# nep-pack/NonlinearEigenproblems.jl

Hardware: AMD Instinct MI355X
Metric: eigenpairs/sec (gun SPMF iar m=100) + compute_Mlincomb GB/s (higher is better)
Workload: dtype f64 (complex128)

## Files before the change

### nonlineareigenproblems.jl_amd/csrc/driver.hip

```cpp
#include "common.h"
#include <vector>
#include <stdlib.h>
#include <time.h>

struct nep_iar {
    nep_spmf* spmf; nep_lu* lu;
    int64_t n, ldv; int32_t m, mt;
    cplx* dV; const cplx* dCtab; int64_t ldc; const int64_t* d_active;
    cplx* dz; cplx* dW;
    std::vector<double> cabs; std::vector<nep_cdouble> cf;
    cplx* dH; nep_cdouble* hH;
    double* d_cabs; cplx* d_ccf;
    cplx* hH_dev;
    int32_t method;
    std::vector<hipEvent_t> ev;
    hipEvent_t e_upload = nullptr; bool upload_waited = false;
    hipStream_t last = nullptr;
    bool no_events = false;
    std::vector<hipGraphExec_t> graphs;
    cplx* dWT = nullptr; int32_t wt_for = 0;
};

extern "C" {

int32_t nep_iar_create(nep_spmf* spmf, nep_lu* lu, int64_t n, int32_t m, nep_cdouble* dV, int64_t ldv,
                       const nep_cdouble* dCtab, int64_t ldc, const int64_t* d_active, nep_cdouble* dwork3n,
                       const double* h_cabs, const nep_cdouble* h_cf, int32_t mt, nep_cdouble* dH, nep_cdouble* h_pinnedH,
                       int32_t orth_method, nep_iar** out) {
    ARGCHK(out != nullptr);
    *out = nullptr;
// ... 94 lines not shown
        rc = nep_iar_shift_scale(n, k, (const nep_cdouble*)col, (nep_cdouble*)vv, stream);
        if (rc) return rc;
    }
    cplx* mirror = s->hH_dev ? s->hH_dev + (int64_t)(k - 1) * (s->m + 4) : nullptr;
    if (s->dWT && k < s->m) {
        rc = nep_orth_dev_iar_next((const nep_cdouble*)s->dV, s->ldv, n, k, s->d_active, (nep_cdouble*)vv, (nep_cdouble*)hrow, s->method,
                                   (nep_cdouble*)mirror, k + 4, (const nep_cdouble*)s->dCtab, s->ldc, s->mt,
                                   (nep_cdouble*)s->dWT, (nep_cdouble*)(vv + s->ldv + n), stream);
        if (!rc) s->wt_for = k + 1;
    } else
        rc = nep_orth_dev_mirror((const nep_cdouble*)s->dV, s->ldv, n * (int64_t)(k + 1), k, s->d_active, (nep_cdouble*)vv,
                                 (nep_cdouble*)hrow, s->method, (nep_cdouble*)mirror, k + 4, stream);
    if (rc) return rc;
    if (!mirror)
        HIPCHK(hipMemcpyAsync(s->hH + (int64_t)(k - 1) * (s->m + 4), hrow, (size_t)(k + 4) * sizeof(cplx), hipMemcpyDeviceToHost, st));
    if (s->no_events) return NEP_OK;
    if (!s->ev[k]) HIPCHK(hipEventCreateWithFlags(&s->ev[k], hipEventDisableTiming | hipEventBlockingSync));
    HIPCHK(hipEventRecord(s->ev[k], st));
    return NEP_OK;
}

int32_t nep_iar_steps(nep_iar* s, int32_t k0, int32_t count, int32_t refine_steps, nep_stream stream) {
    ARGCHK(s && count >= 1);
    for (int32_t k = k0; k < k0 + count; ++k) {
        int rc = nep_iar_step(s, k, refine_steps, stream);
        if (rc) return rc;
    }
    return NEP_OK;
}

int32_t nep_iar_steps_graph(nep_iar* s, int32_t k0, int32_t count, int32_t refine_steps, nep_stream stream, int32_t* captured) {
    ARGCHK(s && count >= 1);
    if (captured) *captured = 0;
// ... 8 lines not shown
        hipGraph_t g = nullptr;
        hipError_t e = hipStreamEndCapture(st, &g);
        hipGraphExec_t ge = nullptr;
        if (!rc && e == hipSuccess && g && hipGraphInstantiate(&ge, g, nullptr, nullptr, 0) == hipSuccess && ge) {
            if (hipGraphLaunch(ge, st) == hipSuccess) { s->graphs.push_back(ge); ok = true; }
            else (void)hipGraphExecDestroy(ge);
        }
        if (g) (void)hipGraphDestroy(g);
        if (!ok) (void)hipGetLastError();
    } else (void)hipGetLastError();
    if (!ok) {
        s->wt_for = wt_for0; s->upload_waited = waited0; s->last = last0;
        return nep_iar_steps(s, k0, count, refine_steps, stream);
    }
    for (int32_t k = k0; k < k0 + count; ++k) {
        if (!s->ev[k]) HIPCHK(hipEventCreateWithFlags(&s->ev[k], hipEventDisableTiming | hipEventBlockingSync));
        HIPCHK(hipEventRecord(s->ev[k], st));
    }
    if (captured) *captured = 1;
    return NEP_OK;
}

int32_t nep_iar_wait(nep_iar* s, int32_t k) {
    ARGCHK(s && k >= 1 && k <= s->m && s->ev[k]);
    for (;;) {
        const hipError_t e = hipEventQuery(s->ev[k]);
        if (e == hipSuccess) return NEP_OK;
        if (e != hipErrorNotReady) HIPCHK(e);
        struct timespec ts = {0, 20000};
        nanosleep(&ts, nullptr);
// ... 11 lines not shown
```

### nonlineareigenproblems.jl_amd/csrc/hesseig.hip

```cpp
#include "common.h"
#include <math.h>

namespace {

constexpr double HQ_ULP = 2.220446049250313e-16;
constexpr double HQ_SAFMIN = 2.2250738585072014e-308;
constexpr int HQ_KMAX = 128;

__host__ __device__ __forceinline__ int hq_off(int c) { return (c * (c + 3)) >> 1; }
__host__ __device__ __forceinline__ int hq_entries(int k) { return hq_off(k - 1) + k; }
__device__ __forceinline__ double cabs1(cplx z) { return fabs(z.x) + fabs(z.y); }
__device__ __forceinline__ cplx readlane_c(cplx v, int lane) { return cmake(readlane_d(v.x, lane), readlane_d(v.y, lane)); }
__device__ __forceinline__ cplx cconj(cplx a) { return cmake(a.x, -a.y); }
__device__ __forceinline__ cplx czero() { return cmake(0.0, 0.0); }

__device__ __forceinline__ double rsqrt_nr(double x) {
    const double y = __builtin_amdgcn_rsq(x);
    const double e = fma(-(x * y), y, 1.0);
    const double q = fma(0.375, e, 0.5);
    return fma(y * e, q, y);
}
__device__ __forceinline__ double rcp_nr(double x) {
    double y = __builtin_amdgcn_rcp(x);
    double e = fma(-x, y, 1.0);
// ... 51 lines not shown
        const double sup = cabs1(A[hq_off(kk) + kk - 1]);
        const double ab = fmax(sub, sup), ba = fmin(sub, sup);
        const double a2 = cabs1(d2), dd = cabs1(csub(d1, d2));
        const double aa = fmax(a2, dd), bb = fmin(a2, dd);
        const double is = rcp_nr(aa + ab);
        if (ba * (ab * is) <= fmax(smlnum, HQ_ULP * (bb * (aa * is)))) return true;
    }
    return false;
}

struct HqCtl {
    int seq;
    int l, i;
    int prog;
    int rq_done;
    int pad[3];
    double tx, ty;
};
typedef __attribute__((address_space(3))) volatile int lds_vint;
typedef __attribute__((address_space(3))) volatile double lds_vdbl;
__device__ __forceinline__ int ctl_load(const int* p) { return *(lds_vint*)p; }
__device__ __forceinline__ void ctl_store(int* p, int v) { *(lds_vint*)p = v; }
__device__ __forceinline__ double ctl_loadd(const double* p) { return *(lds_vdbl*)p; }
__device__ __forceinline__ void ctl_stored(double* p, double v) { *(lds_vdbl*)p = v; }
#define HQ_CBAR() asm volatile("" ::: "memory")

#define HQ_APPLY(c_, s_, up_, lo_, nu_, nl_)                                                                          \
    cplx nu_ = cscale(c_, up_); cfma(nu_, s_, lo_);                                                                   \
    cplx nl_ = cscale(c_, lo_); cfma(nl_, cmake(-(s_).x, (s_).y), up_)

template <bool TWO>
__device__ __forceinline__ void qr_half(cplx* A, cplx* rot, int* prog, const int ld, const int l, const int i,
                                        const int lane) {
    const int c0 = l + lane;
    if (!TWO) {
        const bool in0 = c0 <= i;
        cplx* col = A + hq_off(in0 ? c0 : i);
        cplx up = col[l], lo = col[l + 1];
        cplx lon = col[l + 2];
        double c; cplx s;
        lartg_n(readlane_c(up, 0), readlane_c(lo, 0), c, s);
        cplx pnu, ps; double pc;
        { HQ_APPLY(c, s, up, lo, nu, nl); pnu = nu; pc = c; ps = s; up = nl; lo = lon; }
        for (int j = l + 2; j <= i; ++j) {
            lon = col[j + 1];
            if (in0 && c0 + 2 >= j) col[j - 2] = pnu;
            rot[2 * (j - 1)] = cmake(pc, 0.0); rot[2 * (j - 1) + 1] = ps;
            HQ_CBAR(); ctl_store(prog, j); HQ_CBAR();
// ... 38 lines not shown
        for (int j = jm + 1; j <= i; ++j) {
            lo1n = col1[j + 1];
            if (in1 && c1 + 2 >= j) col1[j - 2] = pnu1;
            rot[2 * (j - 1)] = cmake(pc, 0.0); rot[2 * (j - 1) + 1] = ps;
            HQ_CBAR(); ctl_store(prog, j); HQ_CBAR();
            const int gl = j - 1 - l - 64;
            lartg_n(readlane_c(up1, gl), readlane_c(lo1, gl), c, s);
            HQ_APPLY(c, s, up1, lo1, nu1, nl1);
            pnu1 = nu1; pc = c; ps = s;
            up1 = nl1; lo1 = lo1n;
        }
        if (in1 && c1 + 2 >= i + 1) col1[i - 1] = pnu1;
        rot[2 * i] = cmake(pc, 0.0); rot[2 * i + 1] = ps;
        if (c1 == i) col1[i] = up1;
    }
    HQ_CBAR(); ctl_store(prog, i + 2); HQ_CBAR();
}

#define HQ_RQ(c_, s_, y_, z_, o_, n_)                                                                                 \
    cplx o_ = cscale(c_, y_); cfma_conj(o_, s_, z_);                                              \
    cplx n_ = cscale(c_, z_); cfma(n_, cmake(-(s_).x, -(s_).y), y_)
#define HQ_WAIT(need_)                                                                                                \
    while (pc_ < (need_)) { pc_ = ctl_load(prog); if (pc_ < (need_)) __builtin_amdgcn_s_sleep(1); }                    \
    HQ_CBAR()

template <bool TWO>
__device__ __forceinline__ void rq_half(cplx* A, const cplx* rot, const int* prog, const int ld, const int l, const int i,
                                        const cplx t, const int lane) {
    const int r0 = l + lane;
    int pc_ = 0;
    HQ_WAIT(l + 3);
    if (!TWO) {
        const bool in0 = r0 <= i;
        const int r0c = in0 ? r0 : i;
        cplx y = (lane == 0) ? A[hq_off(l) + l] : czero();
        for (int j = l + 1; j <= i; ++j) {
            HQ_WAIT(j + 2);
            cplx z = A[hq_off(j) + r0c];
            const double c = rot[2 * j].x; const cplx s = rot[2 * j + 1];
            if (r0 > j) z = czero();
            HQ_RQ(c, s, y, z, o, ny);
            if (r0 == j - 1) o = cadd(o, t);
            if (in0 && r0 <= j) A[hq_off((j - 1)) + r0] = o;
            y = ny;
        }
        if (in0) { if (r0 == i) y = cadd(y, t); A[hq_off(i) + r0] = y; }
    } else {
        const int r1 = r0 + 64;
        const bool in1 = r1 <= i;
        const int r1c = in1 ? r1 : i;
        cplx y0 = (lane == 0) ? A[hq_off(l) + l] : czero(), y1 = czero();
        const int jm = l + 63;
        for (int j = l + 1; j <= jm; ++j) {
            HQ_WAIT(j + 2);
            cplx z0 = A[hq_off(j) + r0];
            const double c = rot[2 * j].x; const cplx s = rot[2 * j + 1];
            if (r0 > j) z0 = czero();
            HQ_RQ(c, s, y0, z0, o, ny);
            if (r0 == j - 1) o = cadd(o, t);
            if (r0 <= j) A[hq_off((j - 1)) + r0] = o;
            y0 = ny;
        }
        for (int j = jm + 1; j <= i; ++j) {
            HQ_WAIT(j + 2);
            const cplx z0 = A[hq_off(j) + r0];
            cplx z1 = A[hq_off(j) + r1c];
            const double c = rot[2 * j].x; const cplx s = rot[2 * j + 1];
            if (r1 > j) z1 = czero();
            HQ_RQ(c, s, y0, z0, o0, n0);
            HQ_RQ(c, s, y1, z1, o1, n1);
            if (r0 == j - 1) o0 = cadd(o0, t);
            if (r1 == j - 1) o1 = cadd(o1, t);
            A[hq_off((j - 1)) + r0] = o0;
            if (in1 && r1 <= j) A[hq_off((j - 1)) + r1] = o1;
            y0 = n0; y1 = n1;
        }
        A[hq_off(i) + r0] = y0;
        if (in1) { if (r1 == i) y1 = cadd(y1, t); A[hq_off(i) + r1] = y1; }
    }
}

struct HessWork { cplx* Ht; cplx* wk; cplx* misc; cplx* U; };
__device__ __host__ inline HessWork hq_carve(void* d_work, int k) {
    HessWork W; cplx* p = (cplx*)d_work;
    W.Ht = p; p += (size_t)k * k; W.wk = p; p += k; W.misc = p; p += 2; W.U = p;
    return W;
}

__global__ __launch_bounds__(128) void k_hess_qr(int k0, int kstep, const cplx* __restrict__ H, int64_t ldh, cplx* __restrict__ w_base,
                                                 int64_t w_stride, char* __restrict__ work_base, int64_t work_stride,
                                                 cplx* __restrict__ mirror_base, int64_t mirror_stride) {
    const int k = k0 + (int)blockIdx.x * kstep;
    cplx* __restrict__ w_out = w_base + (size_t)blockIdx.x * w_stride;
    const HessWork Wk = hq_carve(work_base + (size_t)blockIdx.x * work_stride, k);
    cplx* __restrict__ Ht = Wk.Ht; cplx* __restrict__ wk_out = Wk.wk; cplx* __restrict__ misc = Wk.misc;
    cplx* __restrict__ mirror = mirror_base ? mirror_base + (size_t)blockIdx.x * mirror_stride : nullptr;
    extern __shared__ cplx sm[];
    cplx* A = sm;
    cplx* rot = sm + hq_entries(k);
    HqCtl* ctl = (HqCtl*)(rot + 2 * (k + 1));
    const int lane = threadIdx.x & 63;
    const int wave = __builtin_amdgcn_readfirstlane(threadIdx.x >> 6);
    const int ld = k;
    if (threadIdx.x == 0) { ctl->seq = 0; ctl->prog = 0; ctl->rq_done = 0; ctl->l = 0; ctl->i = 0; ctl->tx = 0.0; ctl->ty = 0.0; }
    __syncthreads();
    if (wave == 1) {
        int myseq = 0;
        for (;;) {
            int sq;
            while ((sq = ctl_load(&ctl->seq)) == myseq) __builtin_amdgcn_s_sleep(1);
            HQ_CBAR();
            if (sq < 0) break;
            myseq = sq;
            const int lw = __builtin_amdgcn_readfirstlane(ctl_load(&ctl->l)), iw = __builtin_amdgcn_readfirstlane(ctl_load(&ctl->i));
            const cplx t = cmake(ctl_loadd(&ctl->tx), ctl_loadd(&ctl->ty));
            if (iw - lw + 1 > 64) rq_half<true>(A, rot, &ctl->prog, ld, lw, iw, t, lane);
            else rq_half<false>(A, rot, &ctl->prog, ld, lw, iw, t, lane);
            HQ_CBAR();
            ctl_store(&ctl->rq_done, myseq);
            HQ_CBAR();
        }
        __syncthreads();
        __syncthreads();
        return;
    }
    double amax = 0.0;
    for (int c = 0; c < k; ++c) {
        const int rl = c + 1 < k - 1 ? c + 1 : k - 1;
        for (int r = lane; r <= rl; r += 64) {
            const cplx v = H[(size_t)c * ldh + r];
            A[hq_off(c) + r] = v;
            amax = fmax(amax, fmax(fabs(v.x), fabs(v.y)));
// ... 63 lines not shown
                    cplx y = cscale(s, csqrt_fast(cadd(cmul(xs, xs), cmul(us, us))));
                    if (sx > 0.0 && (x.x * y.x + x.y * y.y) < 0.0) y = cmake(-y.x, -y.y);
                    const cplx den = cadd(x, y);
                    if (den.x != 0.0 || den.y != 0.0) t = csub(t, cmul(u, cdiv_fast(u, den)));
                }
            }
            const int lw = __builtin_amdgcn_readfirstlane(l), iw = __builtin_amdgcn_readfirstlane(i);
            TP(tq3);
            {
                const int d0 = lw + lane, d1 = d0 + 64;
                if (d0 <= iw) A[hq_off(d0) + d0] = csub(A[hq_off(d0) + d0], t);
                if (d1 <= iw) A[hq_off(d1) + d1] = csub(A[hq_off(d1) + d1], t);
            }
            ++seq;
            HQ_CBAR();
            ctl_store(&ctl->prog, 0); ctl_store(&ctl->l, lw); ctl_store(&ctl->i, iw);
            ctl_stored(&ctl->tx, t.x); ctl_stored(&ctl->ty, t.y);
            HQ_CBAR();
            ctl_store(&ctl->seq, seq);
            HQ_CBAR();
            TP(tq4);
            if (iw - lw + 1 > 64) qr_half<true>(A, rot, &ctl->prog, ld, lw, iw, lane);
            else qr_half<false>(A, rot, &ctl->prog, ld, lw, iw, lane);
#ifdef HQ_PROF
            { const long long tq5 = clock64(); tp_wait += tq1 - tq0; tp_scan += tq2 - tq1; tp_shift += tq3 - tq2; tp_pub += tq4 - tq3; tp_qr += tq5 - tq4; tp_steps += iw - lw; }
#endif
        }
        if (!conv) { info = i + 1; break; }
        i = __builtin_amdgcn_readfirstlane(l - 1);
    }
    while (ctl_load(&ctl->rq_done) != seq) __builtin_amdgcn_s_sleep(1);
    HQ_CBAR();
    ctl_store(&ctl->seq, -1);
    HQ_CBAR();
    __syncthreads();
    cplx* wk = rot;
    for (int e = lane; e < k; e += 64) {
        cplx we = czero();
        if (info == 0) { we = A[hq_off(e) + e]; we = cmake(ldexp(we.x, sexp), ldexp(we.y, sexp)); }
        wk[e] = we; w_out[e] = we;
        if (mirror) mirror[e] = we;
    }
    if (info == 0) {
        for (int e = 1; e < k; ++e) {
            for (int guard = 0; guard < 4 * k; ++guard) {
                const cplx we = wk[e];
                bool close = false;
                for (int q = lane; q < e; q += 64) close = close || (cabs1(csub(wk[q], we)) < eps3);
// ... 177 lines not shown
    return NEP_OK;
}

int32_t nep_hess_eigvals_batch_dev(int32_t nb, int32_t k0, int32_t kstep, const nep_cdouble* dH, int64_t ldh, nep_cdouble* d_w,
                                   int64_t w_stride, void* d_work, int64_t work_stride, nep_cdouble* h_mirror,
                                   int64_t mirror_stride, nep_stream stream) {
    ARGCHK(nb >= 1 && k0 >= 1 && kstep >= 0 && dH && d_w && d_work);
    const int kmax = k0 + (nb - 1) * kstep;
    ARGCHK(ldh >= kmax);
    if (kmax > HQ_KMAX) { nep_set_error("nep_hess_eigvals_dev: k = %d exceeds the LDS-resident limit %d", kmax, HQ_KMAX); return NEP_ERR_UNSUPPORTED; }
    if (nb > 1) {
        int64_t need = 0; int rcw = nep_hess_eig_worksize(kmax, &need); if (rcw) return rcw;
        ARGCHK(w_stride >= kmax + 2 && work_stride >= need && (work_stride % 16) == 0 && (!h_mirror || mirror_stride >= kmax + 2));
    }
    const size_t lds = (size_t)16 * hq_entries(kmax) + (size_t)32 * (kmax + 1) + 48;
    if (lds > 65536) { int rc = nep_raise_lds((const void*)k_hess_qr, 163840); if (rc) return rc; }
    cplx* mir = mapped(h_mirror);
    if (h_mirror && !mir) { nep_set_error("nep_hess_eigvals_dev: h_mirror is not mapped pinned host memory"); return NEP_ERR_ARG; }
    hipLaunchKernelGGL(k_hess_qr, dim3((unsigned)nb), dim3(128), lds, as_stream(stream), (int)k0, (int)kstep, (const cplx*)dH, ldh,
                       (cplx*)d_w, w_stride, (char*)d_work, work_stride, mir, mirror_stride);
    LAUNCHCHK();
    return NEP_OK;
}

int32_t nep_hess_eigvecs_batch_dev(int32_t nb, int32_t k0, int32_t kstep, nep_cdouble* d_w, int64_t w_stride, nep_cdouble* dZ,
                                   int64_t ldz, int64_t z_stride, void* d_work, int64_t work_stride, nep_cdouble* h_mirror,
                                   int64_t mirror_stride, nep_stream stream) {
    ARGCHK(nb >= 1 && k0 >= 1 && kstep >= 0 && d_w && dZ && d_work);
    const int kmax = k0 + (nb - 1) * kstep;
    ARGCHK(kmax <= HQ_KMAX && ldz >= kmax && (nb == 1 || z_stride >= (int64_t)kmax * ldz));
    cplx* mir = mapped(h_mirror);
    if (h_mirror && !mir) { nep_set_error("nep_hess_eigvecs_dev: h_mirror is not mapped pinned host memory"); return NEP_ERR_ARG; }
    hipLaunchKernelGGL(k_hess_invit, dim3((unsigned)kmax, (unsigned)nb), dim3(64), 0, as_stream(stream), (int)k0, (int)kstep,
                       (cplx*)d_w, w_stride, (char*)d_work, work_stride, (cplx*)dZ, ldz, z_stride, mir, mirror_stride);
    LAUNCHCHK();
// ... 15 lines not shown
```

### nonlineareigenproblems.jl_amd/csrc/iar_run.hip

```cpp
#include "common.h"
#include <algorithm>
#include <deque>
#include <map>
#include <mutex>
#include <vector>
#include <math.h>
#include <time.h>

extern "C" {
int32_t nep_iar_create(nep_spmf* spmf, nep_lu* lu, int64_t n, int32_t m, nep_cdouble* dV, int64_t ldv, const nep_cdouble* dCtab,
                       int64_t ldc, const int64_t* d_active, nep_cdouble* dwork3n, const double* h_cabs, const nep_cdouble* h_cf,
                       int32_t mt, nep_cdouble* dH, nep_cdouble* h_pinnedH, int32_t orth_method, nep_iar** out);
int32_t nep_iar_steps_graph(nep_iar* s, int32_t k0, int32_t count, int32_t refine_steps, nep_stream stream, int32_t* captured);
}

namespace {

constexpr double EPS = 2.220446049250313e-16;

__global__ void k_iar_active(int64_t* act, int64_t n, int m1) {
    const int j = blockIdx.x * blockDim.x + threadIdx.x;
    if (j < m1) act[j] = (int64_t)(j + 1) * n;
}
__global__ void k_iar_start(cplx* __restrict__ V, const cplx* __restrict__ v, double inv, int64_t n) {
    const int64_t i = (int64_t)blockIdx.x * blockDim.x + threadIdx.x;
    if (i < n) V[i] = cmake(v[i].x * inv, v[i].y * inv);
}

constexpr int64_t ZSLACK = 8192;
__global__ __launch_bounds__(256) void k_iar_zero_slack(cplx* __restrict__ V, int64_t ldv, int64_t n, int m1) {
    const int j = blockIdx.y;
    const int64_t a = (int64_t)(j + 1) * n;
    const int64_t r = a + (int64_t)blockIdx.x * 256 + threadIdx.x;
    if (j < m1 && r < ldv && r < a + ZSLACK) V[(int64_t)j * ldv + r] = cmake(0.0, 0.0);
}

struct RunStreams { hipStream_t check = nullptr, eig = nullptr; hipStream_t probed_for = (hipStream_t)-1; bool shared = false; int retries = 0; };
std::mutex g_rs_mu;
std::map<int, RunStreams> g_rs;

constexpr int RUN_STREAM_CANDIDATES = 8;
int pick_stream(hipStream_t keep, const std::vector<hipStream_t>& others, hipStream_t* out, bool* shared) {
    const int prio = 0, ncand = RUN_STREAM_CANDIDATES;
    std::vector<hipStream_t> cand;
    if (keep) cand.push_back(keep);
    hipStream_t pick = nullptr;
    for (int c = 0; c < ncand && !pick; ++c) {
        hipStream_t s = nullptr;
        if ((size_t)c < cand.size()) s = cand[c];
        else { HIPCHK(hipStreamCreateWithPriority(&s, hipStreamNonBlocking, prio)); cand.push_back(s); }
        bool clash = false;
        for (size_t i = 0; i < others.size() && !clash; ++i) {
            int32_t a = 0;
            int rc = nep_stream_pair_serializes((nep_stream)others[i], (nep_stream)s, &a); if (rc) return rc;
            clash = a != 0;
        }
        if (!clash) pick = s;
    }
    if (getenv("NEP_IAR_RUN_TRACE")) fprintf(stderr, "nep_iar_run: stream pick (prio %d): %zu candidates tried, %s\n", prio, cand.size(), pick ? "free queue found" : "none free");
    if (!pick) { pick = cand[0]; *shared = true; }
    for (hipStream_t s : cand) if (s != pick) (void)hipStreamDestroy(s);
    *out = pick;
    return NEP_OK;
}

int run_streams(hipStream_t main, RunStreams* out) {
    int dev = 0; HIPCHK(hipGetDevice(&dev));
    std::lock_guard<std::mutex> lk(g_rs_mu);
    RunStreams& r = g_rs[dev];
    if (!r.check || !r.eig || r.probed_for != main || (r.shared && r.retries < 3)) {
        if (r.shared) ++r.retries;
        r.shared = false;
        int rc = pick_stream(r.check, {main}, &r.check, &r.shared); if (rc) return rc;
        rc = pick_stream(r.eig, {main, r.check}, &r.eig, &r.shared); if (rc) return rc;
        r.probed_for = main;
    }
    *out = r;
    return NEP_OK;
}

struct Arena {
    int dev = -1; int64_t n = 0; int32_t m = 0, mt = 0;
    cplx* Hdev = nullptr; cplx* wdev = nullptr; cplx* Ctab = nullptr; cplx* work3n = nullptr; int64_t* active = nullptr;
    cplx* v0 = nullptr; double* d_norms = nullptr; void* eigwork = nullptr; int64_t wsz = 0; int bmax = 0;
    cplx* Hpin = nullptr; cplx* wpin = nullptr; double* npin = nullptr; cplx* stage = nullptr;
    void release() {
        for (void* p : {(void*)Hdev, (void*)wdev, (void*)Ctab, (void*)work3n, (void*)active, (void*)v0, (void*)d_norms, eigwork})
            if (p) nep_pool_free(p);
        for (void* p : {(void*)Hpin, (void*)wpin, (void*)npin, (void*)stage}) if (p) (void)hipHostFree(p);
        *this = Arena();
    }
};
std::mutex g_arena_mu;
std::vector<Arena> g_arenas;

int arena_acquire(int64_t n, int32_t m, int32_t mt, int bmax, Arena* out) {
    int dev = 0; HIPCHK(hipGetDevice(&dev));
    {
        std::lock_guard<std::mutex> lk(g_arena_mu);
        for (size_t i = 0; i < g_arenas.size(); ++i)
            if (g_arenas[i].dev == dev && g_arenas[i].n == n && g_arenas[i].m == m && g_arenas[i].mt == mt && g_arenas[i].bmax == bmax) {
                *out = g_arenas[i]; g_arenas.erase(g_arenas.begin() + i); return NEP_OK;
            }
    }
    Arena a; a.dev = dev; a.n = n; a.m = m; a.mt = mt; a.bmax = bmax;
    int64_t wsz = 0; int rc = nep_hess_eig_worksize(m, &wsz); if (rc) return rc;
    a.wsz = (wsz + 15) / 16 * 16;
    void* p = nullptr;
#define AL(dst, type, bytes) do { rc = nep_pool_alloc(&p, (size_t)(bytes)); if (rc) { a.release(); return rc; } dst = (type)p; } while (0)
    AL(a.Hdev, cplx*, (size_t)m * (m + 4) * 16);
    AL(a.wdev, cplx*, (size_t)m * (m + 2) * 16);
    AL(a.Ctab, cplx*, (size_t)m * mt * 16);
    AL(a.work3n, cplx*, (size_t)3 * n * 16);
    AL(a.active, int64_t*, (size_t)(m + 1) * 8);
    AL(a.v0, cplx*, (size_t)n * 16);
    AL(a.d_norms, double*, (size_t)m * 2 * m * 8);
    AL(a.eigwork, void*, (size_t)bmax * a.wsz);
#undef AL
    const size_t stage_bytes = std::max<size_t>((size_t)n * 16, (size_t)m * mt * 16);
    if (hipHostMalloc((void**)&a.Hpin, (size_t)m * (m + 4) * 16, hipHostMallocMapped) != hipSuccess ||
        hipHostMalloc((void**)&a.wpin, (size_t)m * (m + 2) * 16, hipHostMallocMapped) != hipSuccess ||
        hipHostMalloc((void**)&a.npin, (size_t)m * 2 * m * 8, hipHostMallocDefault) != hipSuccess ||
        hipHostMalloc((void**)&a.stage, stage_bytes, hipHostMallocDefault) != hipSuccess) {
        (void)hipGetLastError(); a.release();
        nep_set_error("nep_iar_run: pinned host allocation failed");
        return NEP_ERR_HIP;
    }
    *out = a;
    return NEP_OK;
}
void arena_return(Arena& a) {
    std::lock_guard<std::mutex> lk(g_arena_mu);
// ... 29 lines not shown
            const double om = w[step];
            if (om <= 2.0 * EPS) { ret = step; break; }
            if (om > 0.5 * w_prev) { ret = om > w_prev ? step - 1 : step; break; }
            if (step == umf) { ret = step; break; }
            w_prev = om;
        }
        if (ret < 0) ret = plan;
        last_omega = w[plan];
        recorded = std::max(ret, 1);
        const bool ok = isfinite(w[plan]) && (ret == plan || w[plan] <= std::max(4.0 * EPS, w[ret]));
        if (ok) { if (!hint_off) hint = recorded; } else { hint = -1; hint_off = true; }
        return ok;
    }
};

struct Batch { std::vector<int> kcs; cplx* Zb = nullptr; int kmax = 0; hipEvent_t evW = nullptr, evZ = nullptr; };
struct Check { int kc = 0; std::vector<double> lam; cplx* QT = nullptr; std::vector<double> F; hipEvent_t ev = nullptr; cplx* Zb_owner = nullptr; };

inline cplx hc(const nep_cdouble& z) { cplx r; r.x = z.re; r.y = z.im; return r; }
inline bool ev_done(hipEvent_t e) {
    if (hipEventQuery(e) == hipSuccess) return true;
    (void)hipGetLastError();
    return false;
}

struct Run {
    nep_spmf* spmf; nep_lu* lu; int64_t n; nep_iar_opts o; nep_fv_eval fv; void* ctx; const double* h_fro;
    hipStream_t st; RunStreams rs; Arena a; bool have_arena = false;
    int32_t m, mt; int64_t ldv;
    cplx* V = nullptr; bool own_V = true; nep_iar* step = nullptr;
    Refine ref;
// ... 61 lines not shown
                    const nep_cdouble* h_Ctab, int32_t mt, const double* h_cabs, const nep_cdouble* h_cf, const double* h_fro,
                    nep_fv_eval fv, void* ctx, nep_cdouble* h_lam, nep_cdouble* dQ, nep_cdouble* h_Q, double* h_err,
                    nep_cdouble* dV_basis, nep_iar_result* res, nep_stream stream) {
    ARGCHK(spmf && lu && opts && h_v0 && h_Ctab && fv && h_lam && res);
    ARGCHK(n > 0 && mt >= 1 && opts->maxit >= 1 && opts->check_error_every >= 1);
    ARGCHK(opts->orth_method == 0 || opts->orth_method == 1);
    ARGCHK(opts->errmeasure == 0 || (opts->errmeasure == 1 && h_fro));
    ARGCHK(opts->umfpack_refinements <= 0 || (h_cabs && h_cf));
    memset(res, 0, sizeof(*res));
    res->refine_plan = -1;
    struct timespec t_e_; clock_gettime(CLOCK_MONOTONIC, &t_e_);
    const double t_entry = t_e_.tv_sec * 1e3 + t_e_.tv_nsec * 1e-6;
    const int32_t m = opts->maxit;
    if (m > 128) { nep_set_error("nep_iar_run: maxit = %d exceeds the device eigen-decomposition's limit 128", m); return NEP_ERR_UNSUPPORTED; }
    const int BMAX = std::max(1, nep_env_int("NEP_IAR_EIG_BATCH", 16));
    const int LASTB = std::max(1, nep_env_int("NEP_IAR_EIG_LAST", 8));
    const double T100 = nep_env_double("NEP_IAR_EIG_MS100", 3.3);
    const double TSTEP = 0.35;
    const int cee = opts->check_error_every;
    const double neigs = opts->neigs;
    const bool unthrottled = isinf(neigs) && neigs > 0;

    Run R; R.spmf = spmf; R.lu = lu; R.n = n; R.o = *opts; R.fv = fv; R.ctx = ctx; R.h_fro = h_fro; R.st = as_stream(stream);
    R.m = m; R.mt = mt; R.ldv = n * (int64_t)(m + 1); R.h_err = h_err;
    int rc = run_streams(R.st, &R.rs); if (rc) return rc;
    rc = arena_acquire(n, m, mt, BMAX, &R.a); if (rc) return rc;
    R.have_arena = true;
    Arena& a = R.a;
    hipStream_t st = R.st, cst = R.rs.check, est = R.rs.eig;
    R.ref.umf = opts->umfpack_refinements > 0 ? opts->umfpack_refinements : 0;
    R.ref.hint = (opts->refine_hint >= 0 && nep_env_int("NEP_REFINE_HINT", 1) != 0) ? opts->refine_hint : -1;
    R.filled.assign(m + 1, 0); R.plans.assign(m + 1, 0);
    if (const char* fa = getenv("NEP_IAR_RUN_FAIL_AT")) { if (sscanf(fa, "%d:%d", &R.fail_kind, &R.fail_at) != 2) R.fail_kind = R.fail_at = 0; }
    if (h_err) for (int64_t i = 0; i < (int64_t)m * m; ++i) h_err[i] = NAN;

    if (dV_basis) { R.V = (cplx*)dV_basis; R.own_V = false; }
    else {
        void* p = nullptr;
        rc = nep_pool_alloc(&p, (size_t)(m + 1) * R.ldv * 16); if (rc) return rc;
        R.V = (cplx*)p;
    }
    double nrm2 = 0.0;
    for (int64_t i = 0; i < n; ++i) { a.stage[i] = hc(h_v0[i]); nrm2 += h_v0[i].re * h_v0[i].re + h_v0[i].im * h_v0[i].im; }
    ARGCHK(nrm2 > 0.0 && isfinite(nrm2));
// ... 19 lines not shown
                        (nep_cdouble*)a.Hpin, opts->orth_method, &R.step);
    if (rc) return rc;

    std::vector<char> plan_end(m + 2, 0);
    if (unthrottled) {
        std::vector<int> allk;
        for (int kk = 1; kk <= m; ++kk) if (kk % cee == 0 || kk == m) allk.push_back(kk);
        int e_ = (int)allk.size(); int size = std::min(LASTB, e_);
        while (e_ > 0) {
            plan_end[allk[e_ - 1]] = 1; e_ -= size;
            if (e_ > 0) {
                const double q = allk[e_ - 1] / 100.0;
                size = (int)std::min<double>(std::min(BMAX, e_), std::max(1.0, ceil(2.0 * T100 * q * q / (TSTEP * cee))));
            }
        }
    }
    const bool trace = getenv("NEP_IAR_RUN_TRACE") != nullptr;
    auto now = []() { struct timespec t; clock_gettime(CLOCK_MONOTONIC, &t); return t.tv_sec * 1e3 + t.tv_nsec * 1e-6; };
    double t_fv = 0;
    std::deque<int> pendA; std::deque<Batch> stA; std::deque<Check> stC;
    int slots = unthrottled ? m + 1 : std::max(BMAX, 4);
    const int CHUNK = unthrottled ? 8 : 4;
    const int P = std::min(256, std::max(1, 3072 / mt));
    int k = 1; bool done = false; int status = NEP_OK;
    const bool use_graph = nep_env_flag("NEP_IAR_GRAPH");
    int n_graph = 0;
    auto finished = [&]() { return R.conv >= neigs; };

    auto batch_ready = [&]() -> int {
        if (pendA.empty()) return 0;
        int cnt = 1;
        while (cnt < (int)pendA.size() && cnt < BMAX && pendA[cnt] - pendA[cnt - 1] == pendA[1] - pendA[0] && !(unthrottled && plan_end[pendA[cnt - 1]])) ++cnt;
        if (!unthrottled || plan_end[pendA[cnt - 1]] || cnt >= BMAX || done) return cnt;
        return 0;
    };
    auto launch_batch = [&](int count) -> int {
        Batch b;
        for (int i = 0; i < count; ++i) { b.kcs.push_back(pendA.front()); pendA.pop_front(); }
        const int k0 = b.kcs[0], nb = count; b.kmax = b.kcs.back();
        const int kstep = nb > 1 ? b.kcs[1] - k0 : 0;
        int r = nep_iar_stream_wait(R.step, b.kmax, (nep_stream)est); if (r) return r;
        cplx* wrow = a.wdev + (int64_t)(k0 - 1) * (m + 2);
        cplx* mrow = a.wpin + (int64_t)(k0 - 1) * (m + 2);
        r = nep_hess_eigvals_batch_dev(nb, k0, kstep, (const nep_cdouble*)a.Hdev, m + 4, (nep_cdouble*)wrow, (int64_t)kstep * (m + 2),
                                       a.eigwork, a.wsz, (nep_cdouble*)mrow, (int64_t)kstep * (m + 2), (nep_stream)est);
        if (r) return r;
        b.evW = R.event(); if (!b.evW) return NEP_ERR_HIP;
        HIPCHK(hipEventRecord(b.evW, est));
        void* pz = nullptr;
        r = nep_pool_alloc(&pz, (size_t)nb * b.kmax * b.kmax * 16); if (r) return r;
        b.Zb = (cplx*)pz;
        r = nep_hess_eigvecs_batch_dev(nb, k0, kstep, (nep_cdouble*)wrow, (int64_t)kstep * (m + 2), (nep_cdouble*)b.Zb, b.kmax,
                                       (int64_t)b.kmax * b.kmax, a.eigwork, a.wsz, (nep_cdouble*)mrow, (int64_t)kstep * (m + 2), (nep_stream)est);
        if (r) { nep_pool_free_on(b.Zb, est, true); return r; }
        b.evZ = R.event(); if (!b.evZ) return NEP_ERR_HIP;
        HIPCHK(hipEventRecord(b.evZ, est));
        stA.push_back(b);
        return NEP_OK;
    };
    auto launch_check = [&](const Batch& b, int bi, bool first_of_batch) -> int {
        const int kc = b.kcs[bi];
        int r = R.fill_H(kc); if (r) return r;
        const cplx* w = a.wpin + (int64_t)(kc - 1) * (m + 2);
        if (w[kc].x != 0.0 || (R.fail_kind == 3 && R.fail_at == kc)) { R.retry = 3; nep_set_error("nep_iar_run: the QR iteration of step %d gave up", kc); return NEP_ERR_RETRY; }
        Check c; c.kc = kc; c.lam.resize(2 * (size_t)kc); c.F.resize(2 * (size_t)mt * kc);
        const double sr = R.o.sigma.re, si = R.o.sigma.im, gr = R.o.gamma.re, gi = R.o.gamma.im;
        for (int s = 0; s < kc; ++s) {
            const double dr = w[s].x, di = w[s].y, den = dr * dr + di * di;
// ... 60 lines not shown
            R.s_lam[2 * s] = c.lam[2 * src]; R.s_lam[2 * s + 1] = c.lam[2 * src + 1];
        }
        if (!(kc == m || conv >= neigs)) for (int s = 0; s < nret; ++s) R.s_idx[s] = idx[s];
        if (R.s_QT) nep_pool_free_on(R.s_QT, cst, true);
        R.s_QT = c.QT; c.QT = nullptr; R.s_kq = kc;
        R.conv = conv; R.k_checked = kc;
        R.done(c.ev); c.ev = nullptr;
        return NEP_OK;
    };
    auto drop_check = [&](Check& c) {
        if (c.QT) nep_pool_free_on(c.QT, cst, true);
        if (c.Zb_owner) nep_pool_free_on(c.Zb_owner, cst, true);
        R.done(c.ev);
    };
    auto drop_batch = [&](Batch& b) {
        if (b.Zb) nep_pool_free_on(b.Zb, est, true);
        R.done(b.evW); R.done(b.evZ);
    };

    hipEvent_t te0 = nullptr, te1 = nullptr; bool te1_rec = false;
    if (trace) { (void)hipEventCreate(&te0); (void)hipEventCreate(&te1); (void)hipEventRecord(te0, st); }
    const double t_loop = now();
    double tt_steps = 0, tt_A = 0, tt_B = 0, tt_C = 0, tt_sleep = 0, t_enq_done = 0; double tq = 0;
    while (status == NEP_OK) {
        bool progressed = false;
        tq = now();
        if (!done) {
            if (k <= m && !finished()) {
                int nb = 0;
                while (nb < CHUNK && k + nb <= m) {
                    const bool due = ((k + nb) % cee == 0) || (k + nb == m);
// ... 45 lines not shown
            if (status) { drop_check(c); break; }
        }
        if (status) break;
        if (finished()) {
            done = true; pendA.clear();
            while (!stA.empty()) { drop_batch(stA.front()); stA.pop_front(); }
            while (!stC.empty()) { drop_check(stC.front()); stC.pop_front(); }
        }
        if (trace) { const double t = now(); tt_C += t - tq; tq = t; }
        if (done && pendA.empty() && stA.empty() && stC.empty()) break;
        if (!progressed) { struct timespec ts = {0, 20000}; nanosleep(&ts, nullptr); if (trace) { const double t = now(); tt_sleep += t - tq; tq = t; } }
    }
    if (trace)
        fprintf(stderr, "nep_iar_run trace (ms): set-up %.2f | loop %.2f: steps %.2f (all enqueued at %.2f) A %.2f B %.2f (callback %.2f) C %.2f sleep %.2f\n",
                t_loop - t_entry, now() - t_loop, tt_steps, t_enq_done, tt_A, tt_B, t_fv, tt_C, tt_sleep);
    if (trace && use_graph) fprintf(stderr, "nep_iar_run: %d chunks went out as hipGraphs\n", n_graph);
    if (trace && te0 && te1 && te1_rec) {
        float ms_ = 0.0f;
        if (hipEventSynchronize(te1) == hipSuccess && hipEventElapsedTime(&ms_, te0, te1) == hipSuccess)
            fprintf(stderr, "nep_iar_run: the recurrence's %d steps took %.2f ms on the device\n", m, ms_);
        (void)hipGetLastError();
    }
    if (te0) (void)hipEventDestroy(te0);
    if (te1) (void)hipEventDestroy(te1);
    while (!stA.empty()) { drop_batch(stA.front()); stA.pop_front(); }
    while (!stC.empty()) { drop_check(stC.front()); stC.pop_front(); }
    (void)hipStreamSynchronize(est);
    (void)hipStreamSynchronize(cst);
    res->retry_reason = R.retry;
    res->refine_plan = R.ref.hint_off ? -1 : (R.ref.recorded >= 0 ? R.ref.recorded : R.ref.hint);
    res->refine_hint_off = R.ref.hint_off ? 1 : 0;
    if (status || !unthrottled) (void)hipStreamSynchronize(st);
    if (status) return status;

    int nret = (int)(R.s_lam.size() / 2);
    const bool noconv = (R.conv < neigs) && !unthrottled;
    if (!noconv) nret = std::min(nret, R.conv);
    res->k = R.k_checked > 0 ? R.k_checked : k - 1;
    res->nconv = R.conv; res->nret = nret;
    for (int s = 0; s < nret; ++s) { h_lam[s].re = R.s_lam[2 * s]; h_lam[s].im = R.s_lam[2 * s + 1]; }
    if (nret > 0 && (dQ || h_Q) && R.s_QT) {
        cplx* dst = (cplx*)dQ; void* tmp = nullptr;
// ... 16 lines not shown
```

Baseline: 1417.

## Split Hessenberg QR sweep across four waves and add second eigen stream

The Hessenberg QR kernel gains a four-wave variant. A third wave runs the upper 64-column half of each QR sweep in a pipeline behind the first wave, using a second progress word that the RQ wave waits on. The final eigen-decomposition batch (the one ending at m) now runs on a separate stream with its own workspace, so it can overlap earlier batches, and the default last batch size drops. Per-step event recording is also limited to the steps where a check plan ends, which cuts event overhead. In exchange the kernel carries more inter-wave synchronisation and the arena allocates a larger eigen workspace.

```diff
diff --git a/nonlineareigenproblems.jl_amd/csrc/driver.hip b/nonlineareigenproblems.jl_amd/csrc/driver.hip
--- a/nonlineareigenproblems.jl_amd/csrc/driver.hip
+++ b/nonlineareigenproblems.jl_amd/csrc/driver.hip
@@ -14,6 +14,7 @@
     cplx* hH_dev;
     int32_t method;
     std::vector<hipEvent_t> ev;
+    std::vector<char> ev_steps;
     hipEvent_t e_upload = nullptr; bool upload_waited = false;
     hipStream_t last = nullptr;
     bool no_events = false;
@@ -138,9 +139,15 @@
     if (rc) return rc;
     if (!mirror)
         HIPCHK(hipMemcpyAsync(s->hH + (int64_t)(k - 1) * (s->m + 4), hrow, (size_t)(k + 4) * sizeof(cplx), hipMemcpyDeviceToHost, st));
-    if (s->no_events) return NEP_OK;
+    if (s->no_events || (!s->ev_steps.empty() && !s->ev_steps[k])) return NEP_OK;
     if (!s->ev[k]) HIPCHK(hipEventCreateWithFlags(&s->ev[k], hipEventDisableTiming | hipEventBlockingSync));
     HIPCHK(hipEventRecord(s->ev[k], st));
+    return NEP_OK;
+}
+
+int32_t nep_iar_event_steps(nep_iar* s, const char* steps) {
+    ARGCHK(s && steps);
+    s->ev_steps.assign(steps, steps + s->m + 1);
     return NEP_OK;
 }
 
@@ -179,6 +186,7 @@
         return nep_iar_steps(s, k0, count, refine_steps, stream);
     }
     for (int32_t k = k0; k < k0 + count; ++k) {
+        if (!s->ev_steps.empty() && !s->ev_steps[k]) continue;
         if (!s->ev[k]) HIPCHK(hipEventCreateWithFlags(&s->ev[k], hipEventDisableTiming | hipEventBlockingSync));
         HIPCHK(hipEventRecord(s->ev[k], st));
     }
diff --git a/nonlineareigenproblems.jl_amd/csrc/hesseig.hip b/nonlineareigenproblems.jl_amd/csrc/hesseig.hip
--- a/nonlineareigenproblems.jl_amd/csrc/hesseig.hip
+++ b/nonlineareigenproblems.jl_amd/csrc/hesseig.hip
@@ -89,7 +89,9 @@
     int l, i;
     int prog;
     int rq_done;
-    int pad[3];
+    int prog2;
+    int seq2;
+    int pad;
     double tx, ty;
 };
 typedef __attribute__((address_space(3))) volatile int lds_vint;
@@ -106,7 +108,7 @@
 
 template <bool TWO>
 __device__ __forceinline__ void qr_half(cplx* A, cplx* rot, int* prog, const int ld, const int l, const int i,
-                                        const int lane) {
+                                        const int fin, const int lane) {
     const int c0 = l + lane;
     if (!TWO) {
         const bool in0 = c0 <= i;
@@ -175,28 +177,65 @@
         rot[2 * i] = cmake(pc, 0.0); rot[2 * i + 1] = ps;
         if (c1 == i) col1[i] = up1;
     }
-    HQ_CBAR(); ctl_store(prog, i + 2); HQ_CBAR();
+    HQ_CBAR(); ctl_store(prog, fin); HQ_CBAR();
+}
+
+#define HQ_WAIT(word_, need_)                                                                                         \
+    while (pc_ < (need_)) { pc_ = ctl_load(word_); if (pc_ < (need_)) __builtin_amdgcn_s_sleep(1); }                   \
+    HQ_CBAR()
+
+__device__ __forceinline__ void qr_upper(cplx* A, cplx* rot, const int* prog0, int* prog2, const int l, const int i,
+                                         const int lane) {
+    const int c1 = l + 64 + lane;
+    const bool in1 = c1 <= i;
+    cplx* col1 = A + hq_off(in1 ? c1 : i);
+    cplx up1 = col1[l], lo1 = col1[l + 1], lo1n = col1[l + 2];
+    int pc_ = 0;
+    HQ_WAIT(prog0, l + 2);
+    double c = rot[2 * (l + 1)].x; cplx s = rot[2 * (l + 1) + 1];
+    cplx pnu1, ps; double pc;
+    { HQ_APPLY(c, s, up1, lo1, nu1, nl1); pnu1 = nu1; pc = c; ps = s; up1 = nl1; lo1 = lo1n; }
+    const int jm = l + 64;
+    for (int j = l + 2; j <= jm; ++j) {
+        lo1n = col1[j + 1];
+        if (in1) col1[j - 2] = pnu1;
+        HQ_WAIT(prog0, j + 1);
+        c = rot[2 * j].x; s = rot[2 * j + 1];
+        HQ_APPLY(c, s, up1, lo1, nu1, nl1);
+        pnu1 = nu1; pc = c; ps = s; up1 = nl1; lo1 = lo1n;
+    }
+    for (int j = jm + 1; j <= i; ++j) {
+        lo1n = col1[j + 1];
+        if (in1 && c1 + 2 >= j) col1[j - 2] = pnu1;
+        rot[2 * (j - 1)] = cmake(pc, 0.0); rot[2 * (j - 1) + 1] = ps;
+        HQ_CBAR(); ctl_store(prog2, j); HQ_CBAR();
+        const int gl = j - 1 - l - 64;
+        lartg_n(readlane_c(up1, gl), readlane_c(lo1, gl), c, s);
+        HQ_APPLY(c, s, up1, lo1, nu1, nl1);
+        pnu1 = nu1; pc = c; ps = s;
+        up1 = nl1; lo1 = lo1n;
+    }
+    if (in1 && c1 + 2 >= i + 1) col1[i - 1] = pnu1;
+    rot[2 * i] = cmake(pc, 0.0); rot[2 * i + 1] = ps;
+    if (c1 == i) col1[i] = up1;
+    HQ_CBAR(); ctl_store(prog2, i + 2); HQ_CBAR();
 }
 
 #define HQ_RQ(c_, s_, y_, z_, o_, n_)                                                                                 \
     cplx o_ = cscale(c_, y_); cfma_conj(o_, s_, z_);                                              \
     cplx n_ = cscale(c_, z_); cfma(n_, cmake(-(s_).x, -(s_).y), y_)
-#define HQ_WAIT(need_)                                                                                                \
-    while (pc_ < (need_)) { pc_ = ctl_load(prog); if (pc_ < (need_)) __builtin_amdgcn_s_sleep(1); }                    \
-    HQ_CBAR()
-
-template <bool TWO>
-__device__ __forceinline__ void rq_half(cplx* A, const cplx* rot, const int* prog, const int ld, const int l, const int i,
-                                        const cplx t, const int lane) {
+template <bool TWO, bool FOUR>
+__device__ __forceinline__ void rq_half(cplx* A, const cplx* rot, const int* prog, const int* prog2, const int ld, const int l,
+                                        const int i, const cplx t, const int lane) {
     const int r0 = l + lane;
     int pc_ = 0;
-    HQ_WAIT(l + 3);
+    HQ_WAIT(prog, l + 3);
     if (!TWO) {
         const bool in0 = r0 <= i;
         const int r0c = in0 ? r0 : i;
         cplx y = (lane == 0) ? A[hq_off(l) + l] : czero();
         for (int j = l + 1; j <= i; ++j) {
-            HQ_WAIT(j + 2);
+            HQ_WAIT(prog, j + 2);
             cplx z = A[hq_off(j) + r0c];
             const double c = rot[2 * j].x; const cplx s = rot[2 * j + 1];
             if (r0 > j) z = czero();
@@ -213,7 +252,7 @@
         cplx y0 = (lane == 0) ? A[hq_off(l) + l] : czero(), y1 = czero();
         const int jm = l + 63;
         for (int j = l + 1; j <= jm; ++j) {
-            HQ_WAIT(j + 2);
+            HQ_WAIT(prog, j + 2);
             cplx z0 = A[hq_off(j) + r0];
             const double c = rot[2 * j].x; const cplx s = rot[2 * j + 1];
             if (r0 > j) z0 = czero();
@@ -222,8 +261,10 @@
             if (r0 <= j) A[hq_off((j - 1)) + r0] = o;
             y0 = ny;
         }
+        const int* progb = FOUR ? prog2 : prog;
+        if (FOUR) { HQ_WAIT(prog, i + 2); pc_ = 0; }
         for (int j = jm + 1; j <= i; ++j) {
-            HQ_WAIT(j + 2);
+            HQ_WAIT(progb, j + 2);
             const cplx z0 = A[hq_off(j) + r0];
             cplx z1 = A[hq_off(j) + r1c];
             const double c = rot[2 * j].x; const cplx s = rot[2 * j + 1];
@@ -248,9 +289,11 @@
     return W;
 }
 
-__global__ __launch_bounds__(128) void k_hess_qr(int k0, int kstep, const cplx* __restrict__ H, int64_t ldh, cplx* __restrict__ w_base,
-                                                 int64_t w_stride, char* __restrict__ work_base, int64_t work_stride,
-                                                 cplx* __restrict__ mirror_base, int64_t mirror_stride) {
+template <int WAVES>
+__global__ __launch_bounds__(64 * WAVES) void k_hess_qr(int k0, int kstep, const cplx* __restrict__ H, int64_t ldh, cplx* __restrict__ w_base,
+                                                        int64_t w_stride, char* __restrict__ work_base, int64_t work_stride,
+                                                        cplx* __restrict__ mirror_base, int64_t mirror_stride) {
+    constexpr bool FOUR = WAVES == 4;
     const int k = k0 + (int)blockIdx.x * kstep;
     cplx* __restrict__ w_out = w_base + (size_t)blockIdx.x * w_stride;
     const HessWork Wk = hq_carve(work_base + (size_t)blockIdx.x * work_stride, k);
@@ -263,8 +306,28 @@
     const int lane = threadIdx.x & 63;
     const int wave = __builtin_amdgcn_readfirstlane(threadIdx.x >> 6);
     const int ld = k;
-    if (threadIdx.x == 0) { ctl->seq = 0; ctl->prog = 0; ctl->rq_done = 0; ctl->l = 0; ctl->i = 0; ctl->tx = 0.0; ctl->ty = 0.0; }
+    if (threadIdx.x == 0) {
+        ctl->seq = 0; ctl->prog = 0; ctl->rq_done = 0; ctl->l = 0; ctl->i = 0; ctl->tx = 0.0; ctl->ty = 0.0;
+        ctl->prog2 = 0; ctl->seq2 = 0;
+    }
     __syncthreads();
+    if (FOUR && wave >= 2) {
+        if (wave == 2 && k > 64) {
+            int myseq = 0;
+            for (;;) {
+                int sq;
+                while ((sq = ctl_load(&ctl->seq2)) == myseq) __builtin_amdgcn_s_sleep(2);
+                HQ_CBAR();
+                if (sq < 0) break;
+                myseq = sq;
+                const int lw = __builtin_amdgcn_readfirstlane(ctl_load(&ctl->l)), iw = __builtin_amdgcn_readfirstlane(ctl_load(&ctl->i));
+                qr_upper(A, rot, &ctl->prog, &ctl->prog2, lw, iw, lane);
+            }
+        }
+        __syncthreads();
+        __syncthreads();
+        return;
+    }
     if (wave == 1) {
         int myseq = 0;
         for (;;) {
@@ -275,8 +338,8 @@
             myseq = sq;
             const int lw = __builtin_amdgcn_readfirstlane(ctl_load(&ctl->l)), iw = __builtin_amdgcn_readfirstlane(ctl_load(&ctl->i));
             const cplx t = cmake(ctl_loadd(&ctl->tx), ctl_loadd(&ctl->ty));
-            if (iw - lw + 1 > 64) rq_half<true>(A, rot, &ctl->prog, ld, lw, iw, t, lane);
-            else rq_half<false>(A, rot, &ctl->prog, ld, lw, iw, t, lane);
+            if (iw - lw + 1 > 64) rq_half<true, FOUR>(A, rot, &ctl->prog, &ctl->prog2, ld, lw, iw, t, lane);
+            else rq_half<false, false>(A, rot, &ctl->prog, &ctl->prog2, ld, lw, iw, t, lane);
             HQ_CBAR();
             ctl_store(&ctl->rq_done, myseq);
             HQ_CBAR();
@@ -370,14 +433,18 @@
             }
             ++seq;
             HQ_CBAR();
+            const bool wide = iw - lw + 1 > 64;
             ctl_store(&ctl->prog, 0); ctl_store(&ctl->l, lw); ctl_store(&ctl->i, iw);
+            if (FOUR) ctl_store(&ctl->prog2, 0);
             ctl_stored(&ctl->tx, t.x); ctl_stored(&ctl->ty, t.y);
             HQ_CBAR();
+            if (FOUR && wide) ctl_store(&ctl->seq2, seq);
             ctl_store(&ctl->seq, seq);
             HQ_CBAR();
             TP(tq4);
-            if (iw - lw + 1 > 64) qr_half<true>(A, rot, &ctl->prog, ld, lw, iw, lane);
-            else qr_half<false>(A, rot, &ctl->prog, ld, lw, iw, lane);
+            if (!wide) qr_half<false>(A, rot, &ctl->prog, ld, lw, iw, iw + 2, lane);
+            else if (FOUR) qr_half<false>(A, rot, &ctl->prog, ld, lw, lw + 64, iw + 2, lane);
+            else qr_half<true>(A, rot, &ctl->prog, ld, lw, iw, iw + 2, lane);
 #ifdef HQ_PROF
             { const long long tq5 = clock64(); tp_wait += tq1 - tq0; tp_scan += tq2 - tq1; tp_shift += tq3 - tq2; tp_pub += tq4 - tq3; tp_qr += tq5 - tq4; tp_steps += iw - lw; }
 #endif
@@ -388,6 +455,7 @@
     while (ctl_load(&ctl->rq_done) != seq) __builtin_amdgcn_s_sleep(1);
     HQ_CBAR();
     ctl_store(&ctl->seq, -1);
+    if (FOUR) ctl_store(&ctl->seq2, -1);
     HQ_CBAR();
     __syncthreads();
     cplx* wk = rot;
@@ -595,11 +663,19 @@
         ARGCHK(w_stride >= kmax + 2 && work_stride >= need && (work_stride % 16) == 0 && (!h_mirror || mirror_stride >= kmax + 2));
     }
     const size_t lds = (size_t)16 * hq_entries(kmax) + (size_t)32 * (kmax + 1) + 48;
-    if (lds > 65536) { int rc = nep_raise_lds((const void*)k_hess_qr, 163840); if (rc) return rc; }
+    const int waves = nep_env_int("NEP_HESS_QR_WAVES", 4);
+    if (waves != 2 && waves != 4) { nep_set_error("NEP_HESS_QR_WAVES = %d: 2 or 4", waves); return NEP_ERR_ARG; }
+    const bool four = waves == 4 && kmax > 64;
+    const void* kern = four ? (const void*)k_hess_qr<4> : (const void*)k_hess_qr<2>;
+    if (lds > 65536) { int rc = nep_raise_lds(kern, 163840); if (rc) return rc; }
     cplx* mir = mapped(h_mirror);
     if (h_mirror && !mir) { nep_set_error("nep_hess_eigvals_dev: h_mirror is not mapped pinned host memory"); return NEP_ERR_ARG; }
-    hipLaunchKernelGGL(k_hess_qr, dim3((unsigned)nb), dim3(128), lds, as_stream(stream), (int)k0, (int)kstep, (const cplx*)dH, ldh,
-                       (cplx*)d_w, w_stride, (char*)d_work, work_stride, mir, mirror_stride);
+    if (four)
+        hipLaunchKernelGGL(k_hess_qr<4>, dim3((unsigned)nb), dim3(256), lds, as_stream(stream), (int)k0, (int)kstep, (const cplx*)dH, ldh,
+                           (cplx*)d_w, w_stride, (char*)d_work, work_stride, mir, mirror_stride);
+    else
+        hipLaunchKernelGGL(k_hess_qr<2>, dim3((unsigned)nb), dim3(128), lds, as_stream(stream), (int)k0, (int)kstep, (const cplx*)dH, ldh,
+                           (cplx*)d_w, w_stride, (char*)d_work, work_stride, mir, mirror_stride);
     LAUNCHCHK();
     return NEP_OK;
 }
diff --git a/nonlineareigenproblems.jl_amd/csrc/iar_run.hip b/nonlineareigenproblems.jl_amd/csrc/iar_run.hip
--- a/nonlineareigenproblems.jl_amd/csrc/iar_run.hip
+++ b/nonlineareigenproblems.jl_amd/csrc/iar_run.hip
@@ -12,6 +12,7 @@
                        int64_t ldc, const int64_t* d_active, nep_cdouble* dwork3n, const double* h_cabs, const nep_cdouble* h_cf,
                        int32_t mt, nep_cdouble* dH, nep_cdouble* h_pinnedH, int32_t orth_method, nep_iar** out);
 int32_t nep_iar_steps_graph(nep_iar* s, int32_t k0, int32_t count, int32_t refine_steps, nep_stream stream, int32_t* captured);
+int32_t nep_iar_event_steps(nep_iar* s, const char* steps);
 }
 
 namespace {
@@ -35,7 +36,10 @@
     if (j < m1 && r < ldv && r < a + ZSLACK) V[(int64_t)j * ldv + r] = cmake(0.0, 0.0);
 }
 
-struct RunStreams { hipStream_t check = nullptr, eig = nullptr; hipStream_t probed_for = (hipStream_t)-1; bool shared = false; int retries = 0; };
+struct RunStreams {
+    hipStream_t check = nullptr, eig = nullptr, eig2 = nullptr; hipStream_t probed_for = (hipStream_t)-1; bool shared = false; int retries = 0;
+    bool eig2_probed = false;
+};
 std::mutex g_rs_mu;
 std::map<int, RunStreams> g_rs;
 
@@ -64,17 +68,23 @@
     return NEP_OK;
 }
 
-int run_streams(hipStream_t main, RunStreams* out) {
+int run_streams(hipStream_t main, bool want_eig2, RunStreams* out) {
     int dev = 0; HIPCHK(hipGetDevice(&dev));
     std::lock_guard<std::mutex> lk(g_rs_mu);
     RunStreams& r = g_rs[dev];
     if (!r.check || !r.eig || r.probed_for != main || (r.shared && r.retries < 3)) {
         if (r.shared) ++r.retries;
-        r.shared = false;
+        r.shared = false; r.eig2_probed = false;
         int rc = pick_stream(r.check, {main}, &r.check, &r.shared); if (rc) return rc;
         rc = pick_stream(r.eig, {main, r.check}, &r.eig, &r.shared); if (rc) return rc;
         r.probed_for = main;
     }
+    if (want_eig2 && !r.eig2_probed) {
+        bool sh2 = false;
+        int rc = pick_stream(r.eig2, {main, r.check, r.eig}, &r.eig2, &sh2); if (rc) return rc;
+        if (sh2) { (void)hipStreamDestroy(r.eig2); r.eig2 = nullptr; }
+        r.eig2_probed = true;
+    }
     *out = r;
     return NEP_OK;
 }
@@ -82,7 +92,7 @@
 struct Arena {
     int dev = -1; int64_t n = 0; int32_t m = 0, mt = 0;
     cplx* Hdev = nullptr; cplx* wdev = nullptr; cplx* Ctab = nullptr; cplx* work3n = nullptr; int64_t* active = nullptr;
-    cplx* v0 = nullptr; double* d_norms = nullptr; void* eigwork = nullptr; int64_t wsz = 0; int bmax = 0;
+    cplx* v0 = nullptr; double* d_norms = nullptr; void* eigwork = nullptr; int64_t wsz = 0; int bmax = 0, nsets = 0;
     cplx* Hpin = nullptr; cplx* wpin = nullptr; double* npin = nullptr; cplx* stage = nullptr;
     void release() {
         for (void* p : {(void*)Hdev, (void*)wdev, (void*)Ctab, (void*)work3n, (void*)active, (void*)v0, (void*)d_norms, eigwork})
@@ -94,16 +104,16 @@
 std::mutex g_arena_mu;
 std::vector<Arena> g_arenas;
 
-int arena_acquire(int64_t n, int32_t m, int32_t mt, int bmax, Arena* out) {
+int arena_acquire(int64_t n, int32_t m, int32_t mt, int bmax, int nsets, Arena* out) {
     int dev = 0; HIPCHK(hipGetDevice(&dev));
     {
         std::lock_guard<std::mutex> lk(g_arena_mu);
         for (size_t i = 0; i < g_arenas.size(); ++i)
-            if (g_arenas[i].dev == dev && g_arenas[i].n == n && g_arenas[i].m == m && g_arenas[i].mt == mt && g_arenas[i].bmax == bmax) {
+            if (g_arenas[i].dev == dev && g_arenas[i].n == n && g_arenas[i].m == m && g_arenas[i].mt == mt && g_arenas[i].bmax == bmax && g_arenas[i].nsets == nsets) {
                 *out = g_arenas[i]; g_arenas.erase(g_arenas.begin() + i); return NEP_OK;
             }
     }
-    Arena a; a.dev = dev; a.n = n; a.m = m; a.mt = mt; a.bmax = bmax;
+    Arena a; a.dev = dev; a.n = n; a.m = m; a.mt = mt; a.bmax = bmax; a.nsets = nsets;
     int64_t wsz = 0; int rc = nep_hess_eig_worksize(m, &wsz); if (rc) return rc;
     a.wsz = (wsz + 15) / 16 * 16;
     void* p = nullptr;
@@ -115,7 +125,7 @@
     AL(a.active, int64_t*, (size_t)(m + 1) * 8);
     AL(a.v0, cplx*, (size_t)n * 16);
     AL(a.d_norms, double*, (size_t)m * 2 * m * 8);
-    AL(a.eigwork, void*, (size_t)bmax * a.wsz);
+    AL(a.eigwork, void*, (size_t)nsets * bmax * a.wsz);
 #undef AL
     const size_t stage_bytes = std::max<size_t>((size_t)n * 16, (size_t)m * mt * 16);
     if (hipHostMalloc((void**)&a.Hpin, (size_t)m * (m + 4) * 16, hipHostMallocMapped) != hipSuccess ||
@@ -175,7 +185,7 @@
     }
 };
 
-struct Batch { std::vector<int> kcs; cplx* Zb = nullptr; int kmax = 0; hipEvent_t evW = nullptr, evZ = nullptr; };
+struct Batch { std::vector<int> kcs; cplx* Zb = nullptr; int kmax = 0; hipEvent_t evW = nullptr, evZ = nullptr; hipStream_t es = nullptr; };
 struct Check { int kc = 0; std::vector<double> lam; cplx* QT = nullptr; std::vector<double> F; hipEvent_t ev = nullptr; cplx* Zb_owner = nullptr; };
 
 inline cplx hc(const nep_cdouble& z) { cplx r; r.x = z.re; r.y = z.im; return r; }
@@ -267,7 +277,7 @@
     const int32_t m = opts->maxit;
     if (m > 128) { nep_set_error("nep_iar_run: maxit = %d exceeds the device eigen-decomposition's limit 128", m); return NEP_ERR_UNSUPPORTED; }
     const int BMAX = std::max(1, nep_env_int("NEP_IAR_EIG_BATCH", 16));
-    const int LASTB = std::max(1, nep_env_int("NEP_IAR_EIG_LAST", 8));
+    const bool want2 = nep_env_int("NEP_IAR_EIG_STREAMS", 2) >= 2;
     const double T100 = nep_env_double("NEP_IAR_EIG_MS100", 3.3);
     const double TSTEP = 0.35;
     const int cee = opts->check_error_every;
@@ -276,11 +286,14 @@
 
     Run R; R.spmf = spmf; R.lu = lu; R.n = n; R.o = *opts; R.fv = fv; R.ctx = ctx; R.h_fro = h_fro; R.st = as_stream(stream);
     R.m = m; R.mt = mt; R.ldv = n * (int64_t)(m + 1); R.h_err = h_err;
-    int rc = run_streams(R.st, &R.rs); if (rc) return rc;
-    rc = arena_acquire(n, m, mt, BMAX, &R.a); if (rc) return rc;
+    int rc = run_streams(R.st, want2, &R.rs); if (rc) return rc;
+    const int NES = (want2 && R.rs.eig2) ? 2 : 1;
+    const hipStream_t ests[2] = {R.rs.eig, NES == 2 ? R.rs.eig2 : R.rs.eig};
+    const int LASTB = std::min(BMAX, std::max(1, nep_env_int("NEP_IAR_EIG_LAST", NES == 2 ? 4 : 8)));
+    rc = arena_acquire(n, m, mt, BMAX, NES, &R.a); if (rc) return rc;
     R.have_arena = true;
     Arena& a = R.a;
-    hipStream_t st = R.st, cst = R.rs.check, est = R.rs.eig;
+    hipStream_t st = R.st, cst = R.rs.check;
     R.ref.umf = opts->umfpack_refinements > 0 ? opts->umfpack_refinements : 0;
     R.ref.hint = (opts->refine_hint >= 0 && nep_env_int("NEP_REFINE_HINT", 1) != 0) ? opts->refine_hint : -1;
     R.filled.assign(m + 1, 0); R.plans.assign(m + 1, 0);
@@ -330,6 +343,11 @@
                 size = (int)std::min<double>(std::min(BMAX, e_), std::max(1.0, ceil(2.0 * T100 * q * q / (TSTEP * cee))));
             }
         }
+    }
+    if (unthrottled && nep_env_int("NEP_IAR_STEP_EVENTS", 1) != 0) {
+        std::vector<char> evs(plan_end.begin(), plan_end.begin() + m + 1);
+        if (m % cee != 0 && m > cee) evs[m - m % cee] = 1;
+        rc = nep_iar_event_steps(R.step, evs.data()); if (rc) return rc;
     }
     const bool trace = getenv("NEP_IAR_RUN_TRACE") != nullptr;
     auto now = []() { struct timespec t; clock_gettime(CLOCK_MONOTONIC, &t); return t.tv_sec * 1e3 + t.tv_nsec * 1e-6; };
@@ -350,8 +368,13 @@
         if (!unthrottled || plan_end[pendA[cnt - 1]] || cnt >= BMAX || done) return cnt;
         return 0;
     };
+    int n_batches = 0;
     auto launch_batch = [&](int count) -> int {
         Batch b;
+        ++n_batches;
+        const int set = (NES == 2 && pendA[count - 1] == m) ? 1 : 0;
+        const hipStream_t est = ests[set]; b.es = est;
+        void* const eigwork = (char*)a.eigwork + (size_t)set * BMAX * a.wsz;
         for (int i = 0; i < count; ++i) { b.kcs.push_back(pendA.front()); pendA.pop_front(); }
         const int k0 = b.kcs[0], nb = count; b.kmax = b.kcs.back();
         const int kstep = nb > 1 ? b.kcs[1] - k0 : 0;
@@ -359,7 +382,7 @@
         cplx* wrow = a.wdev + (int64_t)(k0 - 1) * (m + 2);
         cplx* mrow = a.wpin + (int64_t)(k0 - 1) * (m + 2);
         r = nep_hess_eigvals_batch_dev(nb, k0, kstep, (const nep_cdouble*)a.Hdev, m + 4, (nep_cdouble*)wrow, (int64_t)kstep * (m + 2),
-                                       a.eigwork, a.wsz, (nep_cdouble*)mrow, (int64_t)kstep * (m + 2), (nep_stream)est);
+                                       eigwork, a.wsz, (nep_cdouble*)mrow, (int64_t)kstep * (m + 2), (nep_stream)est);
         if (r) return r;
         b.evW = R.event(); if (!b.evW) return NEP_ERR_HIP;
         HIPCHK(hipEventRecord(b.evW, est));
@@ -367,7 +390,7 @@
         r = nep_pool_alloc(&pz, (size_t)nb * b.kmax * b.kmax * 16); if (r) return r;
         b.Zb = (cplx*)pz;
         r = nep_hess_eigvecs_batch_dev(nb, k0, kstep, (nep_cdouble*)wrow, (int64_t)kstep * (m + 2), (nep_cdouble*)b.Zb, b.kmax,
-                                       (int64_t)b.kmax * b.kmax, a.eigwork, a.wsz, (nep_cdouble*)mrow, (int64_t)kstep * (m + 2), (nep_stream)est);
+                                       (int64_t)b.kmax * b.kmax, eigwork, a.wsz, (nep_cdouble*)mrow, (int64_t)kstep * (m + 2), (nep_stream)est);
         if (r) { nep_pool_free_on(b.Zb, est, true); return r; }
         b.evZ = R.event(); if (!b.evZ) return NEP_ERR_HIP;
         HIPCHK(hipEventRecord(b.evZ, est));
@@ -458,7 +481,7 @@
         R.done(c.ev);
     };
     auto drop_batch = [&](Batch& b) {
-        if (b.Zb) nep_pool_free_on(b.Zb, est, true);
+        if (b.Zb) nep_pool_free_on(b.Zb, b.es, true);
         R.done(b.evW); R.done(b.evZ);
     };
 
@@ -534,6 +557,7 @@
     if (trace)
         fprintf(stderr, "nep_iar_run trace (ms): set-up %.2f | loop %.2f: steps %.2f (all enqueued at %.2f) A %.2f B %.2f (callback %.2f) C %.2f sleep %.2f\n",
                 t_loop - t_entry, now() - t_loop, tt_steps, t_enq_done, tt_A, tt_B, t_fv, tt_C, tt_sleep);
+    if (trace) fprintf(stderr, "nep_iar_run: %d decomposition stream(s), %d batches, last batch of %d\n", NES, n_batches, LASTB);
     if (trace && use_graph) fprintf(stderr, "nep_iar_run: %d chunks went out as hipGraphs\n", n_graph);
     if (trace && te0 && te1 && te1_rec) {
         float ms_ = 0.0f;
@@ -545,7 +569,7 @@
     if (te1) (void)hipEventDestroy(te1);
     while (!stA.empty()) { drop_batch(stA.front()); stA.pop_front(); }
     while (!stC.empty()) { drop_check(stC.front()); stC.pop_front(); }
-    (void)hipStreamSynchronize(est);
+    for (int e = 0; e < NES; ++e) (void)hipStreamSynchronize(ests[e]);
     (void)hipStreamSynchronize(cst);
     res->retry_reason = R.retry;
     res->refine_plan = R.ref.hint_off ? -1 : (R.ref.recorded >= 0 ? R.ref.recorded : R.ref.hint);
```

Result: no change. 1425, median of 3 (+0.5%).
